# florasion/D-VQVAE

Hardware: AMD Instinct MI355X
Metric: grasps/sec at batch=65536, N=1024 pts, K=512 (higher is better)
Workload: dtype f32 (GEMMs: every fp32 operand as two fp16 pieces, a1 = fp16(a), a2 = fp16((a - a1) * 2^11), weights pre-scaled by one power of two per output row; the 3 partial products a1 b1, a1 b2, a2 b1 are exact in fp32 and accumulate in TWO fp32 accumulators (large / cross terms) on v_mfma_f32_16x16x32_f16; d

## Files before the change

### d-vqvae_amd/csrc/gemm_f16x2.hip

```cpp
#include "dvq_internal.h"
#include "gemm_common.h"

namespace {

typedef _Float16 h8 __attribute__((ext_vector_type(8)));
typedef _Float16 h2 __attribute__((ext_vector_type(2)));
typedef float f32x2 __attribute__((ext_vector_type(2)));

constexpr int TM = 128, TN = 256, BK = 32;
constexpr int A_PL = TM * 64;
constexpr int W_PL = TN * 64;
constexpr int STAGE = 2 * A_PL + 2 * W_PL;
constexpr float LO_SCALE = 1.0f / 2048.0f;

__device__ __forceinline__ int swz16(int row) { return (4 - ((row >> 2) & 3)) & 3; }

__device__ __forceinline__ void split2(const f32x4& lo, const f32x4& hi, h8& p1, h8& p2) {
    unsigned hb[4], lb[4];
    const float m2048 = -2048.0f;
#pragma unroll
    for (int j = 0; j < 4; ++j) {
        const float a0 = j < 2 ? lo[2 * j] : hi[2 * j - 4], a1 = j < 2 ? lo[2 * j + 1] : hi[2 * j - 3];
        hb[j] = __builtin_bit_cast(unsigned, __builtin_convertvector(f32x2{a0, a1}, h2));
        const float t0 = a0 * 2048.0f, t1 = a1 * 2048.0f;
        asm("v_fma_mixlo_f16 %0, %1, %2, %3 op_sel:[0,0,0] op_sel_hi:[1,0,0]" : "=v"(lb[j]) : "v"(hb[j]), "v"(m2048), "v"(t0));
        asm("v_fma_mixhi_f16 %0, %1, %2, %3 op_sel:[1,0,0] op_sel_hi:[1,0,0]" : "+v"(lb[j]) : "v"(hb[j]), "v"(m2048), "v"(t1));
    }
    p1 = __builtin_bit_cast(h8, uint4{hb[0], hb[1], hb[2], hb[3]});
    p2 = __builtin_bit_cast(h8, uint4{lb[0], lb[1], lb[2], lb[3]});
}

__device__ __forceinline__ f32x4 f16x2_combine(const f32x4& hi, const f32x4& lo, const float* ws, int n, bool vec) {
    f32x4 v = hi + lo * LO_SCALE;
    if (vec) v *= *reinterpret_cast<const f32x4*>(ws + n);
    return v;
}

__device__ __forceinline__ float relu_nan(float x) { return x < 0.f ? 0.f : x; }

template <int EPI>
__device__ __forceinline__ void f16x2_store_block(const GemmParams& p, long m, int n, f32x4 v, bool full) {
    if (full) {
        if (p.bias) v += *reinterpret_cast<const f32x4*>(p.bias + n);
        if constexpr (EPI == EPI_RESID) v += *reinterpret_cast<const f32x4*>(p.resid + m * p.ldr + n);
        if (p.relu) { v[0] = relu_nan(v[0]); v[1] = relu_nan(v[1]); v[2] = relu_nan(v[2]); v[3] = relu_nan(v[3]); }
        *reinterpret_cast<f32x4*>(p.out + m * p.ldo + n) = v;
    } else {
#pragma unroll
        for (int c = 0; c < 4; ++c) {
            if (n + c >= p.N) continue;
            float x = v[c] * p.wscale[n + c] + (p.bias ? p.bias[n + c] : 0.f);
            if constexpr (EPI == EPI_RESID) x += p.resid[m * p.ldr + n + c];
            if (p.relu) x = relu_nan(x);
            p.out[m * p.ldo + n + c] = x;
        }
    }
}

__device__ __forceinline__ float gate_act(float a, float g) {
    const float th = fmaf(-2.0f, __builtin_amdgcn_rcpf(1.0f + __builtin_amdgcn_exp2f(2.8853900817779268f * a)), 1.0f);
    const float sg = __builtin_amdgcn_rcpf(1.0f + __builtin_amdgcn_exp2f(-1.4426950408889634f * g));
    return th * sg;
}

__device__ __forceinline__ void f16x2_store_gate(const GemmParams& p, long m, int na, int c, f32x4 a, f32x4 g, const float* crow) {
    const int nb = na + 32;
    if (p.bias) {
        a += *reinterpret_cast<const f32x4*>(p.bias + na);
        g += *reinterpret_cast<const f32x4*>(p.bias + nb);
    }
    if (p.pre) {
        *reinterpret_cast<f32x4*>(p.pre + m * p.ldpre + na) = a;
        *reinterpret_cast<f32x4*>(p.pre + m * p.ldpre + nb) = g;
    }
    if (crow) {
        a += *reinterpret_cast<const f32x4*>(crow + na);
        g += *reinterpret_cast<const f32x4*>(crow + nb);
    }
    f32x4 o;
#pragma unroll
    for (int q = 0; q < 4; ++q) o[q] = gate_act(a[q], g[q]);
    *reinterpret_cast<f32x4*>(p.out + m * p.ldo + c) = o;
}

__device__ __forceinline__ f32x4 ld4(const float* q) { return *reinterpret_cast<const f32x4*>(q); }
__device__ __forceinline__ void st4(float* q, const f32x4& v) { *reinterpret_cast<f32x4*>(q) = v; }

template <int EPI, int NJ>
__device__ __forceinline__ void f16x2_epilogue_inside(const GemmParams& p, f32x4 (&hi)[NJ][4], f32x4 (&lo)[NJ][4], long m0w, int n0w, int c0w,
                                                      int lane) {
    static_assert(EPI == EPI_BIAS || EPI == EPI_RESID || (EPI == EPI_GATE && NJ == 4), "store epilogues with operands");
    const long m = m0w + (lane & 15);
    const int l4 = 4 * (lane >> 4), nl = n0w + l4;
    f32x4 ws[NJ], bq[NJ], aq[NJ][4];
    const float* crow[4];
#pragma unroll
    for (int jn = 0; jn < NJ; ++jn) ws[jn] = ld4(p.wscale + nl + 16 * jn);
    if (p.bias) {
#pragma unroll
        for (int jn = 0; jn < NJ; ++jn) bq[jn] = ld4(p.bias + nl + 16 * jn);
    }
    if constexpr (EPI == EPI_GATE) {
        if (p.cls) {
#pragma unroll
            for (int i = 0; i < 4; ++i) crow[i] = p.cls + (long)p.label[m + 16 * i] * p.N + nl;
        }
    }
#pragma unroll
    for (int jn = 0; jn < NJ; ++jn)
#pragma unroll
        for (int i = 0; i < 4; ++i) hi[jn][i] = hi[jn][i] + lo[jn][i] * LO_SCALE;
    if constexpr (EPI == EPI_RESID) {
#pragma unroll
        for (int i = 0; i < 4; ++i)
#pragma unroll
            for (int jn = 0; jn < NJ; ++jn) aq[jn][i] = ld4(p.resid + (m + 16 * i) * p.ldr + nl + 16 * jn);
    } else if constexpr (EPI == EPI_GATE) {
        if (p.cls) {
#pragma unroll
            for (int i = 0; i < 4; ++i)
#pragma unroll
                for (int jn = 0; jn < NJ; ++jn) aq[jn][i] = ld4(crow[i] + 16 * jn);
        }
    }
#pragma unroll
    for (int i = 0; i < 4; ++i) {
        if constexpr (EPI == EPI_GATE) {
#pragma unroll
            for (int jn = 0; jn < 2; ++jn) {
                f32x4 a = hi[jn][i] * ws[jn], g = hi[jn + 2][i] * ws[jn + 2];
                if (p.bias) { a += bq[jn]; g += bq[jn + 2]; }
                if (p.pre) {
                    st4(p.pre + (m + 16 * i) * p.ldpre + nl + 16 * jn, a);
                    st4(p.pre + (m + 16 * i) * p.ldpre + nl + 16 * jn + 32, g);
                }
                if (p.cls) { a += aq[jn][i]; g += aq[jn + 2][i]; }
                f32x4 o;
#pragma unroll
                for (int q = 0; q < 4; ++q) o[q] = gate_act(a[q], g[q]);
                st4(p.out + (m + 16 * i) * p.ldo + c0w + l4 + 16 * jn, o);
            }
        } else {
#pragma unroll
            for (int jn = 0; jn < NJ; ++jn) {
                f32x4 v = hi[jn][i] * ws[jn];
                if (p.bias) v += bq[jn];
                if constexpr (EPI == EPI_RESID) v += aq[jn][i];
                if (p.relu) { v[0] = relu_nan(v[0]); v[1] = relu_nan(v[1]); v[2] = relu_nan(v[2]); v[3] = relu_nan(v[3]); }
                st4(p.out + (m + 16 * i) * p.ldo + nl + 16 * jn, v);
            }
        }
    }
}

template <int NJ, bool INIT>
__device__ __forceinline__ void f16x2_init_acc(const GemmParams& p, f32x4 (&hi)[NJ][4], f32x4 (&lo)[NJ][4], long m0w, int n0w, int lane) {
    if constexpr (!INIT) {
#pragma unroll
        for (int a = 0; a < NJ; ++a)
#pragma unroll
            for (int c = 0; c < 4; ++c) { hi[a][c] = f32x4{0.f, 0.f, 0.f, 0.f}; lo[a][c] = f32x4{0.f, 0.f, 0.f, 0.f}; }
        return;
    }
    const int lr = lane & 15, lc = lane >> 4;
    if (p.acc_hi && m0w + 64 <= p.M && n0w + 16 * NJ <= p.N) {
        long r[4];
#pragma unroll
        for (int i = 0; i < 4; ++i) r[i] = m0w + i * 16 + lr;
        if (p.acc_row) {
#pragma unroll
            for (int i = 0; i < 4; ++i) r[i] = p.acc_row[r[i]];
        }
#pragma unroll
        for (int i = 0; i < 4; ++i)
#pragma unroll
            for (int jn = 0; jn < NJ; ++jn) {
                hi[jn][i] = ld4(p.acc_hi + r[i] * p.ldacc + n0w + jn * 16 + 4 * lc);
                lo[jn][i] = ld4(p.acc_lo + r[i] * p.ldacc + n0w + jn * 16 + 4 * lc);
            }
        return;
    }
#pragma unroll
    for (int i = 0; i < 4; ++i) {
        const long m = m0w + i * 16 + lr;
        const bool row_ok = p.acc_hi && m < p.M;
        const long r = row_ok ? (p.acc_row ? p.acc_row[m] : m) : 0;
#pragma unroll
        for (int jn = 0; jn < NJ; ++jn) {
            const int n = n0w + jn * 16 + 4 * lc;
            if (row_ok && n < p.N) {
                hi[jn][i] = *reinterpret_cast<const f32x4*>(p.acc_hi + r * p.ldacc + n);
                lo[jn][i] = *reinterpret_cast<const f32x4*>(p.acc_lo + r * p.ldacc + n);
            } else {
                hi[jn][i] = f32x4{0.f, 0.f, 0.f, 0.f};
                lo[jn][i] = f32x4{0.f, 0.f, 0.f, 0.f};
            }
        }
    }
}

template <int EPI, int NJ = 4>
__device__ __forceinline__ void f16x2_epilogue(const GemmParams& p, f32x4 (&hi)[NJ][4], f32x4 (&lo)[NJ][4], long m0w, int n0w, int c0w,
                                               int lane) {
    static_assert(NJ == 4 || EPI != EPI_GATE, "the gate pairs a wave's tanh columns with their partners 32 columns further");
    if constexpr (EPI == EPI_BIAS || EPI == EPI_RESID || (EPI == EPI_GATE && NJ == 4)) {
        const bool vec_ok = EPI == EPI_GATE || ((p.N % 4 == 0) && (p.ldo % 4 == 0) && (EPI != EPI_RESID || p.ldr % 4 == 0));
        if (vec_ok && m0w + 64 <= p.M && n0w + 16 * NJ <= p.N) {
            f16x2_epilogue_inside<EPI, NJ>(p, hi, lo, m0w, n0w, c0w, lane);
            return;
        }
    }
    const int lr = lane & 15, lc = lane >> 4;
#pragma unroll
    for (int i = 0; i < 4; ++i) {
        const long m = m0w + i * 16 + lr;
        if (m >= p.M) continue;
        if constexpr (EPI == EPI_BIAS || EPI == EPI_RESID) {
            const bool vec_ok = (p.N % 4 == 0) && (p.ldo % 4 == 0) && (EPI != EPI_RESID || p.ldr % 4 == 0);
#pragma unroll
            for (int jn = 0; jn < NJ; ++jn) {
                const int n = n0w + jn * 16 + 4 * lc;
                if (n >= p.N) continue;
                const bool full = vec_ok && n + 3 < p.N;
                f16x2_store_block<EPI>(p, m, n, f16x2_combine(hi[jn][i], lo[jn][i], p.wscale, n, full), full);
            }
        } else if constexpr (EPI == EPI_STATE) {
#pragma unroll
            for (int jn = 0; jn < NJ; ++jn) {
                const int n = n0w + jn * 16 + 4 * lc;
                if (n >= p.N) continue;
                *reinterpret_cast<f32x4*>(p.out + m * p.ldo + n) = hi[jn][i];
                *reinterpret_cast<f32x4*>(p.pre + m * p.ldpre + n) = lo[jn][i];
            }
        } else if constexpr (EPI == EPI_GATE) {
            if constexpr (NJ == 4) {
            if (n0w >= p.N) continue;
            const float* crow = p.cls ? p.cls + (long)p.label[m] * p.N : nullptr;
#pragma unroll
            for (int jn = 0; jn < 2; ++jn) {
                const int nl = jn * 16 + 4 * lc;
                const int na = n0w + nl;
                f16x2_store_gate(p, m, na, c0w + nl, f16x2_combine(hi[jn][i], lo[jn][i], p.wscale, na, true),
                                 f16x2_combine(hi[jn + 2][i], lo[jn + 2][i], p.wscale, na + 32, true), crow);
            }
            }
        }
    }
}

constexpr int PP_STAGES = 3;
constexpr size_t PP_SMEM = PP_STAGES * STAGE;
constexpr size_t PP_SMEM_N128 = PP_STAGES * (2 * A_PL + 2 * 128 * 64);

typedef __attribute__((address_space(3))) char lds_char;
typedef __attribute__((address_space(3))) h8 lds_h8;

template <int V>
struct PpConst { static constexpr int value = V; };

struct PpCursorA {
    int s, tiles;
    const float* a_ptr;
    const float* n_a;
    long n_lda;
    int n_k;
    long n_row;
    const int64_t* nn_arow;
    __device__ __forceinline__ long row(const GemmParams& p, long m0, int tid) const {
        const long m = m0 + (tid >> 2);
        return m < p.M ? m : p.M - 1;
    }
    __device__ __forceinline__ void fetch(const GemmParams& p) {
        const int i1 = min(s + 1, p.nsrc - 1), i2 = min(s + 2, p.nsrc - 1);
        n_a = p.src[i1].A;
        n_lda = p.src[i1].lda;
        n_k = p.src[i1].K;
        nn_arow = p.src[i2].arow;
    }
    __device__ __forceinline__ void open(const GemmParams& p, long m0, int tid) {
        s = 0;
        const GemmSrc& src = p.src[0];
        const long m = row(p, m0, tid);
        const int64_t* arow1 = p.src[min(1, p.nsrc - 1)].arow;
        const long r0 = src.arow ? src.arow[m] : m;
        n_row = arow1 ? arow1[m] : m;
        tiles = (int)((unsigned)src.K / BK);
        a_ptr = src.A + r0 * src.lda + 8 * (tid & 3);
        fetch(p);
    }
    __device__ __forceinline__ void next_source(const GemmParams& p, long m0, int tid) {
        asm volatile("" : "+v"(tid));
        a_ptr = n_a + n_row * n_lda + 8 * (tid & 3);
        tiles = (int)((unsigned)n_k / BK);
        ++s;
        int q = tid >> 2;
        asm volatile("" : "+v"(q) : "v"(a_ptr));
        long m = m0 + q;
        if (m >= p.M) m = p.M - 1;
        n_row = nn_arow ? nn_arow[m] : m;
    }
    __device__ __forceinline__ bool advance(const GemmParams& p, long m0, int tid) {
        a_ptr += BK;
        if (__builtin_expect(--tiles != 0, 1)) return false;
        next_source(p, m0, tid);
        return true;
    }
};

template <int NJ>
struct PpCursorW {
    int s, tiles;
    lds_char* dma_dst[NJ];
    const uint16_t* w_ptr[NJ];
    const uint16_t* n_wp;
    long n_plane, n_ldw;
    int n_k;
    __device__ __forceinline__ void fetch(const GemmParams& p) {
        const int i1 = min(s + 1, p.nsrc - 1);
        n_wp = p.src[i1].Wp;
        n_plane = p.src[i1].wp_plane;
        n_ldw = p.src[i1].ldw;
        n_k = p.src[i1].K;
    }
    __device__ __forceinline__ void place(const GemmParams& p, const uint16_t* wp, long plane, long ldw, int n0, int wave, int lane) {
        const uint16_t* base = wp + (wave >> 2) * plane + 8 * ((lane & 3) ^ swz16(lane >> 2));
        const int nr = n0 + (wave & 3) * (16 * NJ) + (lane >> 2);
#pragma unroll
        for (int i = 0; i < NJ; ++i) w_ptr[i] = base + (long)min(nr + 16 * i, p.N - 1) * ldw;
    }
    __device__ __forceinline__ void open(const GemmParams& p, int n0, int wave, int lane) {
        s = 0;
        const GemmSrc& src = p.src[0];
        tiles = (int)((unsigned)src.K / BK);
        place(p, src.Wp, src.wp_plane, src.ldw, n0, wave, lane);
        fetch(p);
    }
    __device__ __forceinline__ void set_wave(const char* smem, int wave) {
#pragma unroll
        for (int i = 0; i < NJ; ++i) {
            const int id = wave * NJ + i;
            const int pl = id / (4 * NJ), rb = id % (4 * NJ);
            dma_dst[i] = (lds_char*)smem + (2 * A_PL + pl * (64 * NJ * 64) + rb * 1024);
            asm volatile("" : "+s"(dma_dst[i]));
        }
    }
    __device__ __forceinline__ void issue(int stage_off) const {
#pragma unroll
        for (int i = 0; i < NJ; ++i)
            __builtin_amdgcn_global_load_lds((const __attribute__((address_space(1))) void*)w_ptr[i],
                                             (__attribute__((address_space(3))) void*)(dma_dst[i] + stage_off), 16, 0, 0);
    }
    __device__ __forceinline__ bool advance(const GemmParams& p, int n0, int wave, int lane) {
#pragma unroll
        for (int i = 0; i < NJ; ++i) w_ptr[i] += BK;
        if (__builtin_expect(--tiles != 0, 1)) return false;
        asm volatile("" : "+v"(lane));
        place(p, n_wp, n_plane, n_ldw, n0, wave, lane);
        tiles = (int)((unsigned)n_k / BK);
        ++s;
        return true;
    }
};

template <int EPI, int NJ, bool INIT>
__global__ __launch_bounds__(512, 1) void gemm_f16x2_pp_kernel(const GemmParams p, int T) {
    extern __shared__ __attribute__((aligned(16))) char smem_c[];
    constexpr int TN = 64 * NJ, W_PL = TN * 64, STAGE = 2 * A_PL + 2 * W_PL;
    const int tid = threadIdx.x;
    const int tiles_n = (p.N + TN - 1) / TN;
    const long tiles_m = (p.M + TM - 1) / TM;
    const long b = blockIdx.x;
    const long j = b >> 3;
    const long mt = (j / tiles_n) * 8 + (b & 7);
    const int nt = (int)(j % tiles_n);
    if (mt >= tiles_m) return;
    const long m0 = mt * TM;
    const int n0 = nt * TN;
    const int lane = tid & 63;
    const int wave = __builtin_amdgcn_readfirstlane(tid >> 6);
    const int wm = wave >> 2, wn = wave & 3;

    PpCursorA ca;
    PpCursorW<NJ> cw;
    int refetch = 0;
    auto fetch_next = [&]() {
        if (refetch & 1) cw.fetch(p);
        if (refetch & 2) ca.fetch(p);
        refetch = 0;
    };
    cw.open(p, n0, wave, lane);
    cw.set_wave(smem_c, wave);
    const int a_dst = (tid >> 2) * 64 + 16 * ((tid & 3) ^ swz16(tid >> 2));
    f32x4 alo, ahi;
    auto load_a = [&](f32x4& qlo, f32x4& qhi) {
        qlo = *reinterpret_cast<const f32x4*>(ca.a_ptr);
        qhi = *reinterpret_cast<const f32x4*>(ca.a_ptr + 4);
        if (ca.advance(p, m0, tid)) refetch |= 2;
    };
    auto step_w = [&]() {
        if (cw.advance(p, n0, wave, lane)) refetch |= 1;
    };
    auto store_a = [&](lds_char* dst, const f32x4& qlo, const f32x4& qhi) {
        h8 p1, p2;
        split2(qlo, qhi, p1, p2);
        *reinterpret_cast<lds_h8*>(dst) = p1;
        *reinterpret_cast<lds_h8*>(dst + A_PL) = p2;
    };
    char* const st0 = smem_c;
    char* const st1 = smem_c + STAGE;
    cw.issue(0);
    step_w();
    if (refetch) fetch_next();
    if (T > 1) {
        cw.issue(STAGE);
        step_w();
        if (refetch) fetch_next();
    }
    ca.open(p, m0, tid);
    f32x4 a0lo, a0hi, a1lo, a1hi;
    load_a(a0lo, a0hi);
    if (refetch) fetch_next();
    if (T > 1) {
        load_a(a1lo, a1hi);
        if (refetch) fetch_next();
    }
    if (T > 2) {
        load_a(alo, ahi);
        if (refetch) fetch_next();
    }
    store_a((lds_char*)st0 + a_dst, a0lo, a0hi);
    if (T > 1) store_a((lds_char*)st1 + a_dst, a1lo, a1hi);
    asm volatile("s_waitcnt vmcnt(0) lgkmcnt(0)" ::: "memory");
    __builtin_amdgcn_s_barrier();

    f32x4 hi[NJ][4], lo[NJ][4];
    f16x2_init_acc<NJ, INIT>(p, hi, lo, m0 + wm * 64, n0 + wn * 16 * NJ, lane);

    const int rd = (lane & 15) * 64 + 16 * ((lane >> 4) ^ swz16(lane & 15));
    lds_char* fr_a = (lds_char*)smem_c + (wm * 64 * 64 + rd);
    lds_char* fr_w = (lds_char*)smem_c + (2 * A_PL + wn * 16 * NJ * 64 + rd);
    lds_char* wr_a = (lds_char*)smem_c + a_dst;
    asm volatile("" : "+v"(fr_a), "+v"(fr_w), "+v"(wr_a));
    int st_cur = 0, st_n1 = STAGE, st_nx = 2 * STAGE;
    if (wave >= 4) __builtin_amdgcn_s_barrier();
    auto phase_barrier = [&]() __attribute__((always_inline)) {
        __builtin_amdgcn_sched_barrier(0);
        __builtin_amdgcn_s_barrier();
        __builtin_amdgcn_sched_barrier(0);
    };
    auto ktile = [&](auto feed_c) __attribute__((always_inline)) {
        constexpr int FEED = decltype(feed_c)::value;
        if (!(DVQ_DIAG_ON && (p.dbg_abl & 512))) phase_barrier();
        const lds_char* const st_a = fr_a + st_cur;
        const lds_char* const st_w = fr_w + st_cur;
        h8 af[4][2], wf[NJ][2];
#pragma unroll
        for (int i = 0; i < 4; ++i)
#pragma unroll
            for (int pl = 0; pl < 2; ++pl) {
                if (DVQ_DIAG_ON && (p.dbg_abl & 128)) {
                    af[i][pl] = h8{};
                    if (i < NJ) wf[i][pl] = h8{};
                    continue;
                }
                if (DVQ_DIAG_ON && (p.dbg_abl & 64) && pl == 1) {
                    af[i][1] = af[i][0];
                    if (i < NJ) wf[i][1] = wf[i][0];
                    continue;
                }
                af[i][pl] = *reinterpret_cast<const lds_h8*>(st_a + pl * A_PL + i * 16 * 64);
                if (i < NJ) wf[i][pl] = *reinterpret_cast<const lds_h8*>(st_w + pl * W_PL + i * 16 * 64);
            }
        if constexpr (FEED >= 1) asm volatile("s_waitcnt vmcnt(0)" : "+v"(alo), "+v"(ahi) : : "memory");
        else asm volatile("s_waitcnt vmcnt(0)" ::: "memory");
        if constexpr (FEED >= 1) {
            if (!(DVQ_DIAG_ON && (p.dbg_abl & 16))) store_a(wr_a + st_nx, alo, ahi);
            if (!(DVQ_DIAG_ON && (p.dbg_abl & 8))) cw.issue(st_nx);
            if constexpr (FEED == 2) {
                step_w();
                if (!(DVQ_DIAG_ON && (p.dbg_abl & 32))) load_a(alo, ahi);
            }
        }
        asm volatile("s_waitcnt lgkmcnt(0)" ::: "memory");
        phase_barrier();
        __builtin_amdgcn_s_setprio(1);
        if (DVQ_DIAG_ON && (p.dbg_abl & 2)) {
#pragma unroll
            for (int i = 0; i < 4; ++i) asm volatile("" : : "v"(af[i][0]), "v"(af[i][1]), "v"(wf[i < NJ ? i : 0][0]), "v"(wf[i < NJ ? i : 0][1]));
        } else {
#pragma unroll
        for (int jn = 0; jn < NJ; ++jn)
#pragma unroll
            for (int i = 0; i < 4; ++i) hi[jn][i] = __builtin_amdgcn_mfma_f32_16x16x32_f16(wf[jn][0], af[i][0], hi[jn][i], 0, 0, 0);
#pragma unroll
        for (int jn = 0; jn < NJ; ++jn)
#pragma unroll
            for (int i = 0; i < 4; ++i) lo[jn][i] = __builtin_amdgcn_mfma_f32_16x16x32_f16(wf[jn][1], af[i][0], lo[jn][i], 0, 0, 0);
#pragma unroll
        for (int jn = 0; jn < NJ; ++jn)
#pragma unroll
            for (int i = 0; i < 4; ++i) lo[jn][i] = __builtin_amdgcn_mfma_f32_16x16x32_f16(wf[jn][0], af[i][1], lo[jn][i], 0, 0, 0);
        }
        if constexpr (FEED == 2) {
            if (__builtin_expect(refetch != 0, 0)) fetch_next();
        }
        const int st_free = st_cur;
        st_cur = st_n1;
        st_n1 = st_nx;
        st_nx = st_free;
        __builtin_amdgcn_s_setprio(0);
    };
    for (int t = 3; t < T; ++t) ktile(PpConst<2>{});
    if (T > 2) ktile(PpConst<1>{});
    if (T > 1) ktile(PpConst<0>{});
    ktile(PpConst<0>{});
    if (wave < 4) __builtin_amdgcn_s_barrier();
    if (DVQ_DIAG_ON && (p.dbg_abl & 256)) {
        if (hi[0][0][0] + lo[0][0][0] == 12345.678f) p.out[0] = 1.f;
        return;
    }
    f16x2_epilogue<EPI, NJ>(p, hi, lo, m0 + wm * 64, n0 + wn * 16 * NJ, (n0 >> 1) + wn * 32, lane);
}

template <int EPI, int NJ, bool INIT>
int launch_pp(const GemmParams& p, hipStream_t stream) {
    constexpr size_t smem = NJ == 4 ? PP_SMEM : PP_SMEM_N128;
    static DvqOncePerDevice attr_once;
    DVQ_PROPAGATE(dvq_lds_limit(attr_once, reinterpret_cast<const void*>(&gemm_f16x2_pp_kernel<EPI, NJ, INIT>), smem, "gemm_f16x2"));
    const long grid = gemm_padded_grid((p.M + TM - 1) / TM, (p.N + 64 * NJ - 1) / (64 * NJ));
    const double ksum = gemm_ksum(p);
    {
        DVQ_PROF(gemm_prof_name(EPI, p.prof_cls), 2.0 * (double)p.M * p.N * ksum, ((double)p.M + p.N) * ksum * 4, stream);
        DVQ_LAUNCH((gemm_f16x2_pp_kernel<EPI, NJ, INIT>), dim3((unsigned)grid), dim3(512), smem, stream, p, gemm_ktiles(p, BK));
    }
    DVQ_CHECK_LAUNCH("gemm_f16x2");
    return DVQ_OK;
}

template <int EPI, bool INIT = false>
int launch_tiled(const GemmParams& p, hipStream_t stream) {
    if constexpr (EPI != EPI_GATE) {
        const long tiles_m = (p.M + TM - 1) / TM, tiles_n = (p.N + TN - 1) / TN, tiles_n2 = (p.N + 127) / 128, cus = dvq_num_cus();
        const long r256 = (tiles_m * tiles_n + cus - 1) / cus, r128 = (tiles_m * tiles_n2 + cus - 1) / cus;
        bool narrow = r128 < 2 * r256;
        if (dvq_knobs().gemm_tn == 128) narrow = true;
        if (dvq_knobs().gemm_tn == 256) narrow = false;
        if (narrow) return launch_pp<EPI, 2, INIT>(p, stream);
    }
    return launch_pp<EPI, 4, INIT>(p, stream);
}

template <int NB>
struct SkinnySlot {
    uint4 w[NB][2];
    f32x4 a[2];
};

template <int NB>
struct SkinnyCursor16 {
    int s, k_left;
    const float* a_ptr;
    const uint16_t* w_ptr[NB][2];

    __device__ __forceinline__ void open(const GemmParams& p, int src_i, long m, const int (&n)[NB], int lc) {
        s = src_i;
        const GemmSrc& src = p.src[s];
        k_left = src.K;
        a_ptr = src.A + (src.arow ? src.arow[m] : m) * src.lda + 8 * lc;
#pragma unroll
        for (int b = 0; b < NB; ++b)
#pragma unroll
            for (int pl = 0; pl < 2; ++pl) w_ptr[b][pl] = src.Wp + pl * src.wp_plane + (long)n[b] * src.ldw + 8 * lc;
    }
    __device__ __forceinline__ void load(SkinnySlot<NB>& t) const {
#pragma unroll
        for (int b = 0; b < NB; ++b) {
            t.w[b][0] = *reinterpret_cast<const uint4*>(w_ptr[b][0]);
            t.w[b][1] = *reinterpret_cast<const uint4*>(w_ptr[b][1]);
        }
        t.a[0] = *reinterpret_cast<const f32x4*>(a_ptr);
        t.a[1] = *reinterpret_cast<const f32x4*>(a_ptr + 4);
    }
    __device__ __forceinline__ void advance(const GemmParams& p, long m, const int (&n)[NB], int lc, bool last) {
        if (last) return;
        k_left -= BK;
        if (k_left > 0) {
            a_ptr += BK;
#pragma unroll
            for (int b = 0; b < NB; ++b) { w_ptr[b][0] += BK; w_ptr[b][1] += BK; }
        } else open(p, s + 1, m, n, lc);
    }
};

template <int EPI, int R>
__device__ __forceinline__ int skinny_col(int g, int j) {
    if constexpr (EPI == EPI_GATE) {
        constexpr int per64 = 32 / R;
        const int c0 = 64 * (g / per64) + R * (g % per64);
        return j < R ? c0 + j : (j < 2 * R ? c0 + 32 + (j - R) : c0);
    } else {
        return j < R ? R * g + j : R * g;
    }
}

template <int EPI, int R, int NB, int PF>
__device__ __forceinline__ void skinny_body(const GemmParams& p, int T, int groups) {
    const int lane = threadIdx.x;
    const int lr = lane & 15, lc = lane >> 4;
    const long mb0 = (long)blockIdx.y * 16;
    long m = mb0 + lr;
    if (m >= p.M) m = p.M - 1;
    int g[NB], n[NB];
#pragma unroll
    for (int b = 0; b < NB; ++b) {
        g[b] = (int)blockIdx.x * NB + b;
        if (g[b] >= groups) g[b] = groups - 1;
        n[b] = skinny_col<EPI, R>(g[b], lr);
        if (n[b] >= p.N) n[b] = p.N - 1;
    }
    f32x4 hi[NB], lo[NB];
#pragma unroll
    for (int b = 0; b < NB; ++b) {
        hi[b] = f32x4{0.f, 0.f, 0.f, 0.f};
        lo[b] = f32x4{0.f, 0.f, 0.f, 0.f};
        const int nc0 = skinny_col<EPI, R>(g[b], 4 * lc);
        const bool col_live = EPI == EPI_GATE ? 4 * lc < 2 * R : (4 * lc < R && nc0 < p.N);
        if (p.acc_hi && col_live && mb0 + lr < p.M) {
            const long r = p.acc_row ? p.acc_row[mb0 + lr] : mb0 + lr;
            hi[b] = *reinterpret_cast<const f32x4*>(p.acc_hi + r * p.ldacc + nc0);
            lo[b] = *reinterpret_cast<const f32x4*>(p.acc_lo + r * p.ldacc + nc0);
        }
    }
    SkinnyCursor16<NB> cur;
    cur.open(p, 0, m, n, lc);
    SkinnySlot<NB> slot[PF];
    int issued = 0;
#pragma unroll
    for (int u = 0; u < PF; ++u) {
        cur.load(slot[u]);
        cur.advance(p, m, n, lc, issued + 1 >= T);
        issued = issued + 1 < T ? issued + 1 : T;
    }
    for (int t = 0; t < T; t += PF) {
#pragma unroll
        for (int u = 0; u < PF; ++u) {
            if (t + u < T) {
                h8 a1, a2;
                split2(slot[u].a[0], slot[u].a[1], a1, a2);
#pragma unroll
                for (int b = 0; b < NB; ++b) {
                    const h8 w1 = __builtin_bit_cast(h8, slot[u].w[b][0]), w2 = __builtin_bit_cast(h8, slot[u].w[b][1]);
                    hi[b] = __builtin_amdgcn_mfma_f32_16x16x32_f16(w1, a1, hi[b], 0, 0, 0);
                    lo[b] = __builtin_amdgcn_mfma_f32_16x16x32_f16(w2, a1, lo[b], 0, 0, 0);
                    lo[b] = __builtin_amdgcn_mfma_f32_16x16x32_f16(w1, a2, lo[b], 0, 0, 0);
                }
            }
            cur.load(slot[u]);
            cur.advance(p, m, n, lc, issued + 1 >= T);
            issued = issued + 1 < T ? issued + 1 : T;
        }
    }
    const long mo = mb0 + lr;
#pragma unroll
    for (int b = 0; b < NB; ++b) {
        if (b > 0 && (int)blockIdx.x * NB + b >= groups) break;
        const int nc = skinny_col<EPI, R>(g[b], 4 * lc);
        if constexpr (EPI == EPI_GATE) {
            const bool live = 4 * lc < 2 * R && mo < p.M;
            f32x4 v = {0.f, 0.f, 0.f, 0.f};
            if (live) {
                v = f16x2_combine(hi[b], lo[b], p.wscale, nc, true);
                if (p.bias) v += *reinterpret_cast<const f32x4*>(p.bias + nc);
                if (p.pre) *reinterpret_cast<f32x4*>(p.pre + mo * p.ldpre + nc) = v;
                if (p.cls) v += *reinterpret_cast<const f32x4*>(p.cls + (long)p.label[mo] * p.N + nc);
            }
            f32x4 gg;
#pragma unroll
            for (int q = 0; q < 4; ++q) gg[q] = __shfl(v[q], lane + 4 * R, 64);
            if (live && 4 * lc < R) {
                f32x4 o;
#pragma unroll
                for (int q = 0; q < 4; ++q) o[q] = gate_act(v[q], gg[q]);
                const int c = 32 * (nc >> 6) + (nc & 31);
                *reinterpret_cast<f32x4*>(p.out + mo * p.ldo + c) = o;
            }
        } else if constexpr (EPI == EPI_STATE) {
            if (4 * lc >= R || mo >= p.M || nc >= p.N) continue;
            *reinterpret_cast<f32x4*>(p.out + mo * p.ldo + nc) = hi[b];
            *reinterpret_cast<f32x4*>(p.pre + mo * p.ldpre + nc) = lo[b];
        } else {
            if (4 * lc >= R || mo >= p.M || nc >= p.N) continue;
            const bool vec_ok = (p.N % 4 == 0) && (p.ldo % 4 == 0) && (EPI != EPI_RESID || p.ldr % 4 == 0);
            const bool full = vec_ok && nc + 3 < p.N;
            f16x2_store_block<EPI>(p, mo, nc, f16x2_combine(hi[b], lo[b], p.wscale, nc, full), full);
        }
    }
}

template <int EPI, int R, int NB, int PF>
__global__ __launch_bounds__(64) void gemm_f16x2_skinny_kernel(const GemmParams p, int T, int groups) {
    skinny_body<EPI, R, NB, PF>(p, T, groups);
}

struct GemmGroup {
    GemmParams p[DVQ_GEMM_GROUP_MAX];
    int T[DVQ_GEMM_GROUP_MAX];
};
template <int R, int NB, int PF>
__global__ __launch_bounds__(64) void gemm_f16x2_skinny_gate_group_kernel(const GemmGroup g, int groups) {
    skinny_body<EPI_GATE, R, NB, PF>(g.p[blockIdx.z], g.T[blockIdx.z], groups);
}

constexpr long SKINNY_MAX_M = 256;
inline long skinny_max_m(const GemmParams& p) { return p.prof_cls ? 4 * SKINNY_MAX_M : SKINNY_MAX_M; }

template <int EPI>
constexpr int skinny_cols = EPI == EPI_GATE ? 8 : 16;

template <int EPI>
int launch_skinny(const GemmParams& p, hipStream_t stream) {
    constexpr int R = skinny_cols<EPI>;
    const double ksum = gemm_ksum(p);
    const int T = gemm_ktiles(p, BK);
    const int gy = (int)((p.M + 15) / 16);
    const int groups = EPI == EPI_GATE ? (p.N / 64) * (32 / R) : (p.N + R - 1) / R;
    {
        DVQ_PROF(gemm_prof_name(EPI, p.prof_cls), 2.0 * (double)p.M * p.N * ksum, ((double)p.M + p.N) * ksum * 4, stream);
        if (gy >= 3) DVQ_LAUNCH((gemm_f16x2_skinny_kernel<EPI, R, 2, 4>), dim3((unsigned)((groups + 1) / 2), (unsigned)gy), dim3(64), 0, stream, p, T, groups);
        else DVQ_LAUNCH((gemm_f16x2_skinny_kernel<EPI, R, 1, 8>), dim3((unsigned)groups, (unsigned)gy), dim3(64), 0, stream, p, T, groups);
    }
    DVQ_CHECK_LAUNCH("gemm_f16x2_skinny");
    return DVQ_OK;
}

int launch_skinny_gate_group(const GemmParams* ps, int n, hipStream_t stream) {
    constexpr int R = skinny_cols<EPI_GATE>;
    GemmGroup g = {};
    double flops = 0, bytes = 0;
    for (int i = 0; i < n; ++i) {
        g.p[i] = ps[i];
        g.T[i] = gemm_ktiles(ps[i], BK);
        const double ksum = gemm_ksum(ps[i]);
        flops += 2.0 * (double)ps[i].M * ps[i].N * ksum;
        bytes += ((double)ps[i].M + ps[i].N) * ksum * 4;
    }
    const int gy = (int)((ps[0].M + 15) / 16);
    const int groups = (ps[0].N / 64) * (32 / R);
    {
        DVQ_PROF(gemm_prof_name(EPI_GATE, ps[0].prof_cls), flops, bytes, stream);
        if (gy >= 3) DVQ_LAUNCH((gemm_f16x2_skinny_gate_group_kernel<R, 2, 4>), dim3((unsigned)((groups + 1) / 2), (unsigned)gy, (unsigned)n), dim3(64), 0, stream, g, groups);
        else DVQ_LAUNCH((gemm_f16x2_skinny_gate_group_kernel<R, 1, 8>), dim3((unsigned)groups, (unsigned)gy, (unsigned)n), dim3(64), 0, stream, g, groups);
    }
    DVQ_CHECK_LAUNCH("gemm_f16x2_skinny_group");
    return DVQ_OK;
}

__global__ void f16x2_absmax_kernel(const float* __restrict__ w, long rows, int N, int K, float* __restrict__ absmax) {
    const long row = (long)blockIdx.x * (blockDim.x >> 6) + (threadIdx.x >> 6);
    if (row >= rows) return;
    const int lane = threadIdx.x & 63;
    const float* src = w + row * K;
    float mx = 0.f;
    for (int k = lane; k < K; k += 64) {
        const float v = fabsf(src[k]);
        mx = (v > mx || v != v) ? v : mx;
    }
#pragma unroll
    for (int o = 32; o > 0; o >>= 1) {
        const float ov = __shfl_xor(mx, o);
        mx = (ov > mx || ov != ov) ? ov : mx;
    }
    if (lane == 0) {
        atomicMax(reinterpret_cast<unsigned*>(absmax + row % N), __float_as_uint(mx));
    }
}

__device__ __forceinline__ int f16x2_exponent(float amax) {
    if (!(amax > 0.f) || !(amax < INFINITY)) return 0;
    int e;
    (void)frexpf(amax, &e);
    int t = 15 - e;
    if (t > 126) t = 126;
    if (t < -126) t = -126;
    return t;
}

__global__ void f16x2_split_kernel(const float* __restrict__ w, long total, int N, int K, const float* __restrict__ absmax,
                                   uint16_t* __restrict__ planes, float* __restrict__ row_scale) {
    const long i = (long)blockIdx.x * blockDim.x + threadIdx.x;
    if (i >= total) return;
    const int n = (int)((i / K) % N);
    const int t = f16x2_exponent(absmax[n]);
    const float ws = ldexpf(w[i], t);
    const _Float16 h1 = (_Float16)ws;
    const float r = ws - (float)h1;
    const _Float16 h2v = (_Float16)(r * 2048.0f);
    planes[i] = __builtin_bit_cast(uint16_t, h1);
    planes[total + i] = __builtin_bit_cast(uint16_t, h2v);
    if (i < N) row_scale[i] = ldexpf(1.0f, -f16x2_exponent(absmax[i]));
}

}

static int check_f16x2(const GemmParams& p, GemmEpilogue epi) {
    DVQ_REQUIRE(p.wscale, "gemm_f16x2: planes without row scales");
    for (int s = 0; s < p.nsrc; ++s) {
        const GemmSrc& g = p.src[s];
        DVQ_REQUIRE(g.Wp && dvq_aligned16(g.Wp) && g.wp_plane % 8 == 0 && g.ldw % 8 == 0, "gemm_f16x2: weight planes of source %d are not 16-byte aligned", s);
    }
    bool a_ok = true;
    for (int s = 0; s < p.nsrc; ++s) a_ok = a_ok && dvq_aligned16(p.src[s].A) && p.src[s].lda % 4 == 0;
    DVQ_REQUIRE(a_ok, "gemm_f16x2: activation rows are not 16-byte aligned");
    if (epi == EPI_GATE)
        DVQ_REQUIRE(dvq_aligned16(p.out) && p.ldo % 4 == 0 && (!p.pre || (dvq_aligned16(p.pre) && p.ldpre % 4 == 0)), "gemm_f16x2: gate outputs are not 16-byte aligned");
    if (epi == EPI_STATE)
        DVQ_REQUIRE(p.out && p.pre && dvq_aligned16(p.out) && dvq_aligned16(p.pre) && p.ldo % 4 == 0 && p.ldpre % 4 == 0 && p.N % 4 == 0,
                    "gemm_f16x2: accumulator-state outputs need N %% 4 == 0 and 16-byte aligned rows");
    if (p.acc_hi)
        DVQ_REQUIRE(epi == EPI_GATE && p.acc_lo && dvq_aligned16(p.acc_hi) && dvq_aligned16(p.acc_lo) && p.ldacc % 4 == 0 && p.N % 4 == 0,
                    "gemm_f16x2: an accumulator state needs both sums, N %% 4 == 0 and 16-byte aligned rows");
    return DVQ_OK;
}

int dvq_launch_gemm_f16x2_gate_group(const GemmParams* ps, int n, hipStream_t stream) {
    if (!dvq_knobs().gemm_skinny || ps[0].M > skinny_max_m(ps[0])) return -1;
    for (int i = 0; i < n; ++i) DVQ_PROPAGATE(check_f16x2(ps[i], EPI_GATE));
    return launch_skinny_gate_group(ps, n, stream);
}

int dvq_launch_gemm_f16x2(const GemmParams& p, GemmEpilogue epi, hipStream_t stream) {
    DVQ_PROPAGATE(check_f16x2(p, epi));
#ifdef DVQ_DIAG
    if (const char* e = getenv("DVQ_GEMM_ABL")) const_cast<GemmParams&>(p).dbg_abl = atoi(e);
#endif
    if (dvq_knobs().gemm_skinny && p.M <= skinny_max_m(p)) switch (epi) {
        case EPI_BIAS: return launch_skinny<EPI_BIAS>(p, stream);
        case EPI_RESID: return launch_skinny<EPI_RESID>(p, stream);
        case EPI_GATE: return launch_skinny<EPI_GATE>(p, stream);
        case EPI_STATE: return launch_skinny<EPI_STATE>(p, stream);
        default: break;
    }
    switch (epi) {
        case EPI_BIAS: return launch_tiled<EPI_BIAS>(p, stream);
        case EPI_RESID: return launch_tiled<EPI_RESID>(p, stream);
        case EPI_GATE: return p.acc_hi ? launch_tiled<EPI_GATE, true>(p, stream) : launch_tiled<EPI_GATE, false>(p, stream);
        case EPI_STATE: return launch_tiled<EPI_STATE>(p, stream);
        default: break;
    }
    dvq_set_error("gemm_f16x2: epilogue %d is not available on the fp16 split path", (int)epi);
    return DVQ_EINVAL;
}

extern "C" int dvq_f16x2_row_absmax(const float* w, int64_t outer, int N, int K, float* row_absmax, dvq_stream_t stream) {
    DVQ_REQUIRE(outer >= 1 && N >= 1 && K >= 1 && w && row_absmax, "f16x2_row_absmax: bad arguments");
    const long rows = (long)outer * N;
    DVQ_LAUNCH(f16x2_absmax_kernel, dim3((unsigned)((rows + 3) / 4)), dim3(256), 0, (hipStream_t)stream, w, rows, N, K, row_absmax);
    DVQ_CHECK_LAUNCH("f16x2_row_absmax");
    return DVQ_OK;
}

extern "C" int dvq_split_f16x2(const float* w, int64_t outer, int N, int K, const float* row_absmax, uint16_t* planes, float* row_scale,
                               dvq_stream_t stream) {
    DVQ_REQUIRE(outer >= 1 && N >= 1 && K >= 1 && w && row_absmax && planes && row_scale, "split_f16x2: bad arguments");
    const long total = (long)outer * N * K;
    DVQ_LAUNCH(f16x2_split_kernel, dim3((unsigned)((total + 255) / 256)), dim3(256), 0, (hipStream_t)stream, w, total, N, K, row_absmax, planes,
               row_scale);
    DVQ_CHECK_LAUNCH("split_f16x2");
    return DVQ_OK;
}
```

Measured before the change: 204,700.

## Store fp16 weight planes K-tiled so each BK slab of all rows is contiguous

The weight split kernel now writes the fp16 planes in a [K/BK][N][BK] tiled layout, so each BK-wide slab across all output rows is one contiguous block. The pipelined GEMM cursor keeps a single tile base pointer plus 32-bit per-row offsets, advancing by N*BK per tile instead of updating NJ 64-bit pointers. The skinny path is updated to the same layout. It also requires ldw == K. The intent is fewer address registers and VALU work per tile and more contiguous DMA fetches, but a K that is not a multiple of BK silently falls back to the row-major layout, which the GEMM paths no longer index correctly.

Result: faster. 209,200 (median of 6 runs) (+2.2%).

```diff
diff --git a/d-vqvae_amd/csrc/gemm_f16x2.hip b/d-vqvae_amd/csrc/gemm_f16x2.hip
--- a/d-vqvae_amd/csrc/gemm_f16x2.hip
+++ b/d-vqvae_amd/csrc/gemm_f16x2.hip
@@ -311,28 +311,26 @@
 struct PpCursorW {
     int s, tiles;
     lds_char* dma_dst[NJ];
-    const uint16_t* w_ptr[NJ];
+    const uint16_t* w_tile;
+    unsigned w_off[NJ];
     const uint16_t* n_wp;
-    long n_plane, n_ldw;
+    long n_plane;
     int n_k;
     __device__ __forceinline__ void fetch(const GemmParams& p) {
         const int i1 = min(s + 1, p.nsrc - 1);
         n_wp = p.src[i1].Wp;
         n_plane = p.src[i1].wp_plane;
-        n_ldw = p.src[i1].ldw;
         n_k = p.src[i1].K;
-    }
-    __device__ __forceinline__ void place(const GemmParams& p, const uint16_t* wp, long plane, long ldw, int n0, int wave, int lane) {
-        const uint16_t* base = wp + (wave >> 2) * plane + 8 * ((lane & 3) ^ swz16(lane >> 2));
-        const int nr = n0 + (wave & 3) * (16 * NJ) + (lane >> 2);
-#pragma unroll
-        for (int i = 0; i < NJ; ++i) w_ptr[i] = base + (long)min(nr + 16 * i, p.N - 1) * ldw;
     }
     __device__ __forceinline__ void open(const GemmParams& p, int n0, int wave, int lane) {
         s = 0;
         const GemmSrc& src = p.src[0];
         tiles = (int)((unsigned)src.K / BK);
-        place(p, src.Wp, src.wp_plane, src.ldw, n0, wave, lane);
+        w_tile = src.Wp + (wave >> 2) * src.wp_plane;
+        const int nr = n0 + (wave & 3) * (16 * NJ) + (lane >> 2);
+        const int chunk = 8 * ((lane & 3) ^ swz16(lane >> 2));
+#pragma unroll
+        for (int i = 0; i < NJ; ++i) w_off[i] = 2u * (unsigned)(min(nr + 16 * i, p.N - 1) * BK + chunk);
         fetch(p);
     }
     __device__ __forceinline__ void set_wave(const char* smem, int wave) {
@@ -344,18 +342,18 @@
             asm volatile("" : "+s"(dma_dst[i]));
         }
     }
-    __device__ __forceinline__ void issue(int stage_off) const {
+    __device__ __forceinline__ void issue(int stage_off) {
+#pragma unroll
+        for (int i = 0; i < NJ; ++i) asm volatile("" : "+v"(w_off[i]));
 #pragma unroll
         for (int i = 0; i < NJ; ++i)
-            __builtin_amdgcn_global_load_lds((const __attribute__((address_space(1))) void*)w_ptr[i],
+            __builtin_amdgcn_global_load_lds((const __attribute__((address_space(1))) void*)(reinterpret_cast<const char*>(w_tile) + w_off[i]),
                                              (__attribute__((address_space(3))) void*)(dma_dst[i] + stage_off), 16, 0, 0);
     }
-    __device__ __forceinline__ bool advance(const GemmParams& p, int n0, int wave, int lane) {
-#pragma unroll
-        for (int i = 0; i < NJ; ++i) w_ptr[i] += BK;
+    __device__ __forceinline__ bool advance(const GemmParams& p, int wave) {
+        w_tile += (long)p.N * BK;
         if (__builtin_expect(--tiles != 0, 1)) return false;
-        asm volatile("" : "+v"(lane));
-        place(p, n_wp, n_plane, n_ldw, n0, wave, lane);
+        w_tile = n_wp + (wave >> 2) * n_plane;
         tiles = (int)((unsigned)n_k / BK);
         ++s;
         return true;
@@ -398,7 +396,7 @@
         if (ca.advance(p, m0, tid)) refetch |= 2;
     };
     auto step_w = [&]() {
-        if (cw.advance(p, n0, wave, lane)) refetch |= 1;
+        if (cw.advance(p, wave)) refetch |= 1;
     };
     auto store_a = [&](lds_char* dst, const f32x4& qlo, const f32x4& qhi) {
         h8 p1, p2;
@@ -570,7 +568,7 @@
 #pragma unroll
         for (int b = 0; b < NB; ++b)
 #pragma unroll
-            for (int pl = 0; pl < 2; ++pl) w_ptr[b][pl] = src.Wp + pl * src.wp_plane + (long)n[b] * src.ldw + 8 * lc;
+            for (int pl = 0; pl < 2; ++pl) w_ptr[b][pl] = src.Wp + pl * src.wp_plane + (long)n[b] * BK + 8 * lc;
     }
     __device__ __forceinline__ void load(SkinnySlot<NB>& t) const {
 #pragma unroll
@@ -587,7 +585,7 @@
         if (k_left > 0) {
             a_ptr += BK;
 #pragma unroll
-            for (int b = 0; b < NB; ++b) { w_ptr[b][0] += BK; w_ptr[b][1] += BK; }
+            for (int b = 0; b < NB; ++b) { w_ptr[b][0] += (long)p.N * BK; w_ptr[b][1] += (long)p.N * BK; }
         } else open(p, s + 1, m, n, lc);
     }
 };
@@ -795,8 +793,10 @@
     const _Float16 h1 = (_Float16)ws;
     const float r = ws - (float)h1;
     const _Float16 h2v = (_Float16)(r * 2048.0f);
-    planes[i] = __builtin_bit_cast(uint16_t, h1);
-    planes[total + i] = __builtin_bit_cast(uint16_t, h2v);
+    const int k = (int)(i % K);
+    const long j = K % BK ? i : i - ((long)n * K + k) + ((long)(k / BK) * N + n) * BK + k % BK;
+    planes[j] = __builtin_bit_cast(uint16_t, h1);
+    planes[total + j] = __builtin_bit_cast(uint16_t, h2v);
     if (i < N) row_scale[i] = ldexpf(1.0f, -f16x2_exponent(absmax[i]));
 }
 
@@ -807,6 +807,7 @@
     for (int s = 0; s < p.nsrc; ++s) {
         const GemmSrc& g = p.src[s];
         DVQ_REQUIRE(g.Wp && dvq_aligned16(g.Wp) && g.wp_plane % 8 == 0 && g.ldw % 8 == 0, "gemm_f16x2: weight planes of source %d are not 16-byte aligned", s);
+        DVQ_REQUIRE(g.ldw == g.K, "gemm_f16x2: the fp16 image of source %d is the whole [N=%d][K=%d] block of dvq_split_f16x2 (ldw=%ld)", s, p.N, g.K, g.ldw);
     }
     bool a_ok = true;
     for (int s = 0; s < p.nsrc; ++s) a_ok = a_ok && dvq_aligned16(p.src[s].A) && p.src[s].lda % 4 == 0;
```
